# fukangl/SMG-multimodal-grasping

Hardware: AMD Instinct MI355X
Metric: affordance fwd+bwd passes/sec (16-rot 224^2 RGB-D) (higher is better)
Workload: dtype f32; 1 GPU; 16 rot x 224^2 (S=640): fwd + Huber + bwd + Adam per GPU per step; reinforcement_net style 0; 17 trunk passes; fp32; leg=headline, rotations=16, input_size=640, parallelism=dp1

## Files before the change

smg-multimodal-grasping_amd/csrc/backward.hip:

```cpp
#include "engine.h"

int do_backward(smg_engine* e, const smg_net* net, const float* dq, hipStream_t st, int phases, bool elem_head) {
    if (!e->have_fwd) return fail(-22, "smg_backward without a preceding smg_forward");
    if (!net->grads) return fail(-22, "net.grads is NULL");
    if (phases == 2 && !e->bw_phase0_done)
        return fail(-22, "smg_backward_phase(1) must follow smg_backward_phase(0) of the same forward");
    if ((phases & 1) && e->bw_phase0_done)
        return fail(-22, "smg_backward / smg_backward_phase(0) while the second half of a two-phase backward is still due (run phase 1 or a new forward)");
    const Layout& L = *e->L;
    const TrunkRef& T = L.trunk[e->f_trunk];
    const HeadRef& Hd = L.head[e->f_head];
    const int NS = e->f_streams, NP = e->f_pairs;
    const float* P = net->params;
    float* Gr = net->grads;
    const Plane p4 = e->p_blk[3];
    const bool ph_a = phases & 1, ph_b = phases & 2;
    if (ph_a) {
        for (int r = 0; r < kStatRep; ++r) HIP_OK(hipMemsetAsync(e->bstat + (size_t)r * kStatRepStride, 0, 2 * e->bstat_span * sizeof(double), st));
    }
    const bool split16 = e->prec == 0 && kSplitOp == 3;
    if (ph_a && split16) HIP_OK(hipMemsetAsync(e->gamax, 0, (size_t)e->gamax_words * sizeof(unsigned), st));
    const hipStream_t s2 = (e->prof || e->serialize) ? st : e->side;
    auto fork = [&](hipEvent_t ev) -> int {
        HIP_OK(hipEventRecord(ev, st));
// ... 52 lines not shown
        p.bbuf = e->F; p.ldb = 2 * kFeat; p.pb = p4; p.NB = 2 * kFeat;
        p.bsum = fsum(e, e->st_F); p.bsq = fsq(e, e->st_F); p.bstride = 2 * kFeat; p.bgamma = P + Hd.n0.w; p.bbeta = P + Hd.n0.b;
        p.eps = kEps; p.chunk = chunk4; p.chunks_per_stream = cps4; p.n_chunks = NP * cps4;
        p.dw = Gr + Hd.c0.w; p.ldw_out = 2 * kFeat;
        if (fork(e->ev_misc)) return -5;
        const dim3 grid(1, 2 * kFeat / 64, NP * cps4);
        return launch_wgrad(e, s2, p, grid, K_HW0, 2.0 * NP * p4.HW * 2 * kFeat * kHeadMid,
                            4.0 * NP * p4.HW * (2 * kHeadMid + 2 * kFeat), 1, C_IDENT, tiles, tiles.place_alone(wgrad_partial_floats(p, grid)));
        };
        PREC_DISPATCH(e, if (int rc = go(PTAG)) return rc);
    }
    {
        auto run = [&](auto tag, auto ptag) {
                using Cfg = decltype(tag);
                BwdDataP<Cfg, false, E_STORE, true, decltype(ptag)::value, true> p{};
        p.gbuf = e->DH1; p.ldg = kHeadMid; p.gcoff = 0; p.xbuf = e->H1; p.ldx = kHeadMid; p.xcoff = 0; p.pa = p4; p.KA = kHeadMid;
        p.xsum = fsum(e, e->st_H1); p.xsq = fsq(e, e->st_H1); p.xstride = kHeadMid;
        p.s1 = b1(e, e->st_H1); p.s2 = b2(e, e->st_H1); p.sstride = kHeadMid; p.scoff = 0; p.agamma = P + Hd.n1.w;
        p.wp = e->packed_u + e->pk_hd0; p.K8tot = kHeadMid / 8; p.ldn = 2 * kFeat; p.wcol0 = 0; p.N = 2 * kFeat;
        p.mbuf = e->F; p.ldm = 2 * kFeat; p.mcoff = 0; p.pm = p4;
        p.msum = fsum(e, e->st_F); p.msq = fsq(e, e->st_F); p.mstride = 2 * kFeat; p.egamma = P + Hd.n0.w; p.ebeta = P + Hd.n0.b;
        p.dst = e->DF; p.ldd = 2 * kFeat; p.dcoff = 0;
        p.o1 = b1(e, e->st_F); p.o2 = b2(e, e->st_F); p.ostride = 2 * kFeat; p.ocoff = 0;
        p.dbeta = Gr + Hd.n0.b; p.dgamma = Gr + Hd.n0.w; p.rep_stride = 0; p.eps = kEps;
        launch_gemm(e, st, p, dim3(NP * p4.HWp / Cfg::BM, 2 * kFeat / Cfg::BN), K_HD0, 2.0 * NP * p4.HW * 2 * kFeat * kHeadMid,
                    4.0 * NP * p4.HW * (2 * kHeadMid + 2 * 2 * kFeat));
            };
            PREC_DISPATCH(e, if (p4.HWp % 128 == 0) run(CfgP128x128{}, PTAG); else run(CfgP64x128{}, PTAG));
    }
    {
        Norm5BwdArgs a;
        a.DF = e->DF; a.F = e->F; a.p4 = p4; a.fsum = fsum(e, e->st_F); a.fsq = fsq(e, e->st_F);
        a.f1 = b1(e, e->st_F); a.f2 = b2(e, e->st_F); a.hgamma = P + Hd.n0.w;
        a.x4 = e->X[3]; a.xsum = fsum(e, e->st_X[3]); a.xsq = fsq(e, e->st_X[3]); a.gamma5 = P + T.norm5.w; a.eps = kEps;
        a.user_ptr = e->d_user_ptr; a.user_pair = e->d_user_pair; a.user_slot = e->d_user_slot;
        a.G4 = e->G[3]; a.SA = b1(e, e->st_X[3]); a.SB = b2(e, e->st_X[3]);
        a.dbeta5 = Gr + T.norm5.b; a.dgamma5 = Gr + T.norm5.w; a.chunk = 16;
        PREC_DISPATCH(e, launch_kernel(e, norm5_bwd_kernel<PREC>, dim3(4, NS, (p4.HW + 15) / 16), dim3(256), 0, st, K_OTHER, 0, 0, false, a));
    }
    }
    struct LayerBuf { float* GS; float* D2; float* D2S; int ring; };
    auto buf_of = [&](int b, int i) -> LayerBuf {
        const int r = ring_pos(b, i);
        return LayerBuf{e->GS[r % kRing], e->D2[r % kRing], e->D2S[r % kRing], r};
    };
    auto fused_gsrc = [&](int b, const DenseLayerRef& d) {
        const int Ct = kBlockCtot[b];
        GradSrc g{};
        g.g = el(e, e->G[b], d.cin); g.ldg = Ct; g.x = el(e, e->X[b], d.cin); g.ldx = Ct;
        g.xsum = fsum(e, e->st_X[b]) + d.cin; g.xsq = fsq(e, e->st_X[b]) + d.cin;
        g.s1 = b1(e, e->st_X[b]) + d.cin; g.s2 = b2(e, e->st_X[b]) + d.cin; g.sstride = Ct; g.eps = kEps;
        return g;
    };
    auto issue_wgrads = [&](int b, int i) -> int {
        const Plane pl = e->p_blk[b];
        const int Ct = kBlockCtot[b];
        const DenseLayerRef& d = T.layers[b][i];
        float* bt = el(e, e->Bt, e->bt_off[b][i]);
        const LayerBuf lb = buf_of(b, i);
        const WgradPlan w = plan_layer_wgrads(pl, d.cin, NS, e->prec, split16, e->deterministic, e->part_floats, e->generic3x3, e->generic_w1);
        GradSrc gsrc{};
        if (gs_on_side(pl)) launch_gs_apply(b, i, s2, lb.GS);
        if (gs_materialised) { gsrc.g = lb.GS; gsrc.ldg = kGrowth; gsrc.amax = gamax_of(e, b, i, 0); }
        else gsrc = fused_gsrc(b, d);
        if (!e->generic3x3) {
            const PartialTiles::Slot at = tiles.place_halo3x3(w.w3.groups);
            if (at.refused) return fail(-12, tiles.refusal());
            launch_reduce2(e, s2, at.first);
            Halo3x3WgradArgs a;
            a.g = gsrc; a.pl = pl; a.src = bt; a.C = kBottleneck;
            a.bt = bn_table(e, e->sb_tab[b][i], e->max_streams, 0, kBottleneck, P + d.n2.w, P + d.n2.b);
            a.asc = asc_n2(e, b, i);
            a.tiles_x = w.w3.tiles_x; a.n_tiles = w.w3.n_tiles; a.tiles_per_wg = w.w3.tiles_per_wg;
            a.part = part_at(e, at);
            a.groups = w.w3.groups; a.streams = NS;
            const double flops = 2.0 * NS * pl.HW * 9 * kBottleneck * kGrowth, bytes = ESZ(e) * NS * pl.HW * (kGrowth + kBottleneck);
            if (w.w3.ts == 16) {
                PREC_DISPATCH(e, launch_kernel(e, conv3x3_halo_wgrad_kernel<16, PREC>, dim3(w.w3_grid), dim3(256), HaloWgradSGeo<16, PREC>::smem_bytes(), s2,
                                               K_W3, flops, bytes, false, a));
            } else {
                PREC_DISPATCH(e, launch_kernel(e, conv3x3_halo_wgrad_kernel<8, PREC>, dim3(w.w3_grid), dim3(256), HaloWgradSGeo<8, PREC>::smem_bytes(), s2,
                                               K_W3, flops, bytes, false, a));
            }
            launch_reduce2(e, s2, tiles.launched(at, reduce_tap_inner(a.part, w.w3.groups * NS, Gr + d.c2.w)));
        } else {
            int chunk, cps;
            pick_chunk(pl, NS, 9, chunk, cps);
            BwdWeightP<CfgW32x128, W_THREE, C_3x3, kPdWgrad, false> p{};
            p.gbuf = lb.GS; p.ldg = kGrowth; p.gcoff = 0; p.xbuf = nullptr; p.pa = pl; p.MA = kGrowth;
            p.bbuf = bt; p.ldb = kBottleneck; p.pb = pl; p.NB = kBottleneck;
            p.bsum = fsum(e, e->st_Bt[b][i]); p.bsq = fsq(e, e->st_Bt[b][i]); p.bstride = kBottleneck;
            p.bgamma = P + d.n2.w; p.bbeta = P + d.n2.b; p.eps = kEps;
            p.chunk = chunk; p.chunks_per_stream = cps; p.n_chunks = NS * cps;
            p.dw = Gr + d.c2.w; p.ldw_out = kBottleneck * 9;
            const dim3 grid(1, 1, 9 * NS * cps);
            if (int rc = launch_wgrad(e, s2, p, grid, K_W3, 2.0 * NS * pl.HW * 9 * kBottleneck * kGrowth,
                                      ESZ(e) * NS * pl.HW * (kGrowth + kBottleneck), 9, C_3x3, tiles, tiles.place_alone(wgrad_partial_floats(p, grid)))) return rc;
        }
        if (w.w1_ws) {
            using G = WswGeo;
            static_assert(G::BN == kW1WsTileN, "plan_layer_wgrads counts this kernel's column tiles");
            Wgrad1x1WsArgs a{};
            a.d2 = reinterpret_cast<const u32x4*>(lb.D2); a.binv = lb.D2S; a.x = e->X[b]; a.ldb = Ct; a.pl = pl; a.NB = d.cin;
            a.btab = stat_table(e, e->sx_tab[b], e->max_streams, Ct); a.bgamma = P + d.n1.w; a.bbeta = P + d.n1.b; a.basc = asc_n1(e, b, i);
            a.chunk = w.chunk; a.chunks_per_stream = w.cps; a.n_chunks = NS * w.cps;
            a.dw = Gr + d.c1.w; a.ldw_out = d.cin; a.ldp = w.nt * G::BN;
            const PartialTiles::Slot at = tiles.place_behind3x3((int64_t)a.n_chunks * G::BM * a.ldp);
            launch_reduce2(e, s2, at.first);
            if (at.refused) return fail(-12, tiles.refusal());
            a.part = part_at(e, at);
            a.tm = TileMap{a.n_chunks, w.nt, 0};
            launch_kernel(e, conv1x1_wgrad_ws_kernel, dim3(tile_grid(a.tm)), dim3(512), G::smem_bytes(w.chunk), s2, K_W1,
                          2.0 * NS * pl.HW * d.cin * kBottleneck, 4.0 * NS * pl.HW * (kBottleneck + d.cin), false, a);
            ReduceArgs red1{};
            if (a.part) red1 = reduce_chunk_major(a.part, a.n_chunks, 1, G::BM, d.cin, G::BM, a.ldp, a.dw, d.cin, C_IDENT);
            launch_reduce2(e, s2, tiles.launched(at, red1));
        } else {
            using Cfg = CfgW128x64;
            static_assert(Cfg::BN == kW1TileN, "plan_layer_wgrads counts this kernel's column tiles");
            auto go = [&](auto ptag) -> int {
                BwdWeightP<MC<Cfg, decltype(ptag)::value>, W_ONE, C_IDENT, kPdWgrad, false, decltype(ptag)::value> p{};
                p.gbuf = lb.D2; p.ldg = kBottleneck; p.gcoff = 0; p.xbuf = nullptr; p.pa = pl; p.MA = kBottleneck; p.binv = lb.D2S; p.basc = asc_n1(e, b, i);
                p.bbuf = e->X[b]; p.ldb = Ct; p.pb = pl; p.NB = d.cin;
                p.bsum = fsum(e, e->st_X[b]); p.bsq = fsq(e, e->st_X[b]); p.bstride = Ct; p.btab = stat_table(e, e->sx_tab[b], e->max_streams, Ct);
                p.bgamma = P + d.n1.w; p.bbeta = P + d.n1.b; p.eps = kEps;
                p.chunk = w.chunk; p.chunks_per_stream = w.cps; p.n_chunks = NS * w.cps;
                p.dw = Gr + d.c1.w; p.ldw_out = d.cin;
                const dim3 grid(1, w.nt, NS * w.cps);
                return launch_wgrad(e, s2, p, grid, K_W1, 2.0 * NS * pl.HW * d.cin * kBottleneck,
                                    ESZ(e) * NS * pl.HW * (kBottleneck + d.cin), 1, C_IDENT, tiles, tiles.place_behind3x3(wgrad_partial_floats(p, grid)));
            };
            PREC_DISPATCH(e, if (int rc = go(PTAG)) return rc);
        }
        return 0;
    };
    auto debug_stop = [&]() -> int {
        launch_reduce2(e, s2, tiles.drain());
        HIP_OK(hipEventRecord(e->ev_end, s2));
        HIP_OK(hipStreamWaitEvent(st, e->ev_end, 0));
        if (int rc = walk_status(e)) return rc;
        e->have_fwd = false; e->bw_phase0_done = false; e->prof_stage = -1;
        return 0;
    };
    const bool pooled_tail = e->prec == 0 && e->f_stem1 && !e->stem_plane_tail && (NS > 4 || e->deterministic);
    for (int b = ph_a ? 3 : 0; b >= (ph_b ? 0 : 1); --b) {
        e->prof_stage = b;
        const Plane pl = e->p_blk[b];
        const int Ct = kBlockCtot[b];
        if (e->dbg_stop == b * 100 + 50) return debug_stop();
        if (b == 0 && pooled_tail) {
            StemMomArgs a;
            a.img = e->img4; a.pi = e->p_img; a.ps = e->p_stem; a.part = e->mom_part;
// ... 27 lines not shown
                const double flops = 2.0 * NS * pl.HW * 9 * kBottleneck * kGrowth;
                const double bytes = ESZ(e) * NS * pl.HW * (kGrowth + 2 * kBottleneck);
                if (halo_tile(pl, NS) == 16) {
                    a.tiles_x = (pl.W + 15) / 16; a.cg_per_wg = kBottleneck / 32;
                    if (pl.H % 16 || pl.W % 16) {
                        PREC_DISPATCH(e, launch_kernel(e, conv3x3_halo_dgrad_kernel<16, PREC, true>, dim3(((pl.H + 15) / 16) * a.tiles_x, NS), dim3(256),
                                                       HaloDgradSGeo<16, PREC>::smem_bytes(kBottleneck), st, K_D3, flops, bytes, true, a));
                    } else {
                        PREC_DISPATCH(e, launch_kernel(e, conv3x3_halo_dgrad_kernel<16, PREC>, dim3((pl.H / 16) * a.tiles_x, NS), dim3(256),
                                                       HaloDgradSGeo<16, PREC>::smem_bytes(kBottleneck), st, K_D3, flops, bytes, true, a));
                    }
                } else {
                    a.tiles_x = (pl.W + 7) / 8; a.cg_per_wg = 1;
                    PREC_DISPATCH(e, launch_kernel(e, conv3x3_halo_dgrad_kernel<8, PREC>, dim3(((pl.H + 7) / 8) * a.tiles_x, NS, kBottleneck / 64), dim3(256),
                                                   HaloDgradSGeo<8, PREC>::smem_bytes(kBottleneck), st, K_D3, flops, bytes, true, a));
                }
            } else {
                auto run = [&](auto tag) {
                    using Cfg = decltype(tag);
                    BwdDataP<Cfg, true, E_STORE, false> p{};
                    p.gbuf = GSb; p.ldg = kGrowth; p.gcoff = 0; p.xbuf = nullptr; p.pa = pl; p.KA = kGrowth;
                    p.wp = e->packed_u + e->pk_g3d[b][i]; p.K8tot = 9 * kGrowth / 8; p.ldn = kBottleneck; p.wcol0 = 0; p.N = kBottleneck;
                    p.mbuf = bt; p.ldm = kBottleneck; p.mcoff = 0; p.pm = pl;
                    p.msum = fsum(e, e->st_Bt[b][i]); p.msq = fsq(e, e->st_Bt[b][i]); p.mstride = kBottleneck;
                    p.egamma = P + d.n2.w; p.ebeta = P + d.n2.b;
                    p.dst = split16 ? e->DY2 : D2b; p.ldd = kBottleneck; p.dcoff = 0;
                    p.o1 = b1(e, e->st_Bt[b][i]); p.o2 = b2(e, e->st_Bt[b][i]); p.ostride = kBottleneck; p.ocoff = 0;
                    p.dbeta = Gr + d.n2.b; p.dgamma = Gr + d.n2.w; p.eps = kEps;
                    launch_gemm(e, st, p, dim3(NS * pl.HWp / Cfg::BM, kBottleneck / Cfg::BN), K_D3, 2.0 * NS * pl.HW * 9 * kBottleneck * kGrowth,
                                ESZ(e) * NS * pl.HW * (kGrowth + 2 * kBottleneck));
                };
                if (pl.HWp % 128 == 0) run(CfgP128x128{}); else run(CfgP64x128{});
            }
            if (split16) {
                BnBwdApplySplitArgs a{};
                a.g = e->DY2; a.x = bt; a.pl = pl;
                a.xsum = fsum(e, e->st_Bt[b][i]); a.xsq = fsq(e, e->st_Bt[b][i]); a.xstride = kBottleneck; a.xtab = !e->generic3x3 ? stat_table(e, e->sb_tab[b][i], e->max_streams, kBottleneck) : StatTab{};
                a.s1 = b1(e, e->st_Bt[b][i]); a.s2 = b2(e, e->st_Bt[b][i]); a.sstride = kBottleneck;
                a.gamma = P + d.n2.w; a.eps = kEps; a.out = reinterpret_cast<u32x4*>(D2b); a.binv = lb.D2S;
                if (!e->generic3x3) { a.dbeta = Gr + d.n2.b; a.dgamma = Gr + d.n2.w; }
                launch_kernel(e, bn_bwd_apply_split_kernel, dim3(pl.HWp / kScaleBlock, NS), dim3(256), 0, st, K_OTHER, 0, 4.0 * NS * pl.HW * 3 * kBottleneck, false, a);
            } else {
                BnBwdApplyArgs a{};
                a.g = D2b; a.ldg = kBottleneck; a.gcoff = 0; a.x = bt; a.ldx = kBottleneck; a.xcoff = 0; a.pl = pl; a.C = kBottleneck;
                a.xsum = fsum(e, e->st_Bt[b][i]); a.xsq = fsq(e, e->st_Bt[b][i]); a.xstride = kBottleneck; a.xtab = !e->generic3x3 ? stat_table(e, e->sb_tab[b][i], e->max_streams, kBottleneck) : StatTab{};
                a.s1 = b1(e, e->st_Bt[b][i]); a.s2 = b2(e, e->st_Bt[b][i]); a.sstride = kBottleneck; a.scoff = 0;
                a.gamma = P + d.n2.w; a.eps = kEps; a.out = D2b; a.ldo = kBottleneck; a.amax = nullptr;
                if (!e->generic3x3) { a.dbeta = Gr + d.n2.b; a.dgamma = Gr + d.n2.w; }
                PREC_DISPATCH(e, launch_kernel(e, bn_bwd_apply_kernel<PREC>, dim3((pl.HWp + bn_apply_rows(PREC) - 1) / bn_apply_rows(PREC), NS), dim3(256), 0, st,
                                               K_OTHER, 0, ESZ(e) * NS * pl.HW * 3 * kBottleneck, false, a));
            }
            if (fork(e->ev_d2[lb.ring % kRing])) return -5;
            if (int rc = issue_wgrads(b, i)) return rc;
            HIP_OK(hipEventRecord(e->ev_side[lb.ring % kRing], s2));
            if (e->dbg_stop == b * 100 + i && e->prec == 0) {
                const int64_t nf = (int64_t)NS * pl.HWp * Ct;
                if (e->dbg_gsnap_floats < nf) {
                    if (e->dbg_gsnap) (void)hipFree(e->dbg_gsnap);
                    e->dbg_gsnap = nullptr; e->dbg_gsnap_floats = 0;
                    HIP_OK(hipMalloc((void**)&e->dbg_gsnap, (size_t)nf * sizeof(float)));
                    e->dbg_gsnap_floats = nf;
                }
                HIP_OK(hipMemcpyAsync(e->dbg_gsnap, e->G[b], (size_t)nf * sizeof(float), hipMemcpyDeviceToDevice, st));
            }
            const int L = (int)T.layers[b].size();
            const int g_lo = i - ((L - 1 - i) % kGroup == kGroup - 1 ? 0 : std::min(i, kGroup - 1 - (L - 1 - i) % kGroup));
            const int cs = T.layers[b][g_lo].cin;
            if (d.cin > cs) {
                auto run = [&](auto tag, auto ptag) {
                    using Cfg = MC<decltype(tag), decltype(ptag)::value>;
                    BwdDataP<Cfg, false, E_ACCUM, false, decltype(ptag)::value> p{};
                    p.gbuf = D2b; p.ldg = kBottleneck; p.gcoff = 0; p.xbuf = nullptr; p.pa = pl; p.KA = kBottleneck; p.binv = lb.D2S;
                    p.wp = e->packed_u + e->pk_d1[b][i]; p.K8tot = kBottleneck / 8; p.ldn = d.cin; p.wcol0 = cs; p.N = d.cin - cs;
                    p.mbuf = e->X[b]; p.ldm = Ct; p.mcoff = cs; p.pm = pl;
                    p.msum = fsum(e, e->st_X[b]); p.msq = fsq(e, e->st_X[b]); p.mstride = Ct; p.mtab = stat_table(e, e->sx_tab[b], e->max_streams, Ct);
                    p.egamma = P + d.n1.w + cs; p.ebeta = P + d.n1.b + cs;
                    p.dst = e->G[b]; p.ldd = Ct; p.dcoff = cs;
                    p.o1 = b1(e, e->st_X[b]); p.o2 = b2(e, e->st_X[b]); p.ostride = Ct; p.ocoff = cs;
                    p.dbeta = e->dbscr + e->db_off[b][i] + cs; p.dgamma = e->dbscr + e->db_off[b][i] + d.cin + cs; p.rep_stride = e->db_total; p.eps = kEps;
                    launch_gemm(e, st, p, dim3(NS * pl.HWp / Cfg::BM, (p.N + Cfg::BN - 1) / Cfg::BN), K_D1, 2.0 * NS * pl.HW * p.N * kBottleneck,
                                ESZ(e) * NS * pl.HW * (kBottleneck + 3.0 * p.N));
                };
                PREC_DISPATCH(e, if (pl.HWp % 128 == 0) run(CfgP128x64{}, PTAG); else run(CfgP64x64{}, PTAG));
            }
            if (i == g_lo) {
                auto run = [&](auto tag, auto ptag) {
                    using Cfg = MC<decltype(tag), decltype(ptag)::value>;
                    BwdDataGroupP<Cfg, decltype(ptag)::value> p{};
                    const int g_hi = L - 1 - ((L - 1 - g_lo) / kGroup) * kGroup;
                    p.nseg = g_hi - g_lo + 1;
                    for (int k = 0; k < p.nseg; ++k) {
                        const DenseLayerRef& dk = T.layers[b][g_lo + k];
                        const LayerBuf lk = buf_of(b, g_lo + k);
                        p.seg[k].g = lk.D2; p.seg[k].wp = e->packed_u + e->pk_d1[b][g_lo + k]; p.seg[k].ldn = dk.cin; p.seg[k].binv = lk.D2S;
                        p.seg[k].gamma = P + dk.n1.w; p.seg[k].beta = P + dk.n1.b;
                        p.seg[k].dbeta = e->dbscr + e->db_off[b][g_lo + k]; p.seg[k].dgamma = e->dbscr + e->db_off[b][g_lo + k] + dk.cin;
                    }
                    p.ldg = kBottleneck; p.pa = pl; p.KA = kBottleneck; p.N = cs;
                    p.mbuf = e->X[b]; p.ldm = Ct;
                    p.msum = fsum(e, e->st_X[b]); p.msq = fsq(e, e->st_X[b]); p.mstride = Ct; p.mtab = stat_table(e, e->sx_tab[b], e->max_streams, Ct);
                    p.dst = e->G[b]; p.ldd = Ct;
                    p.o1 = b1(e, e->st_X[b]); p.o2 = b2(e, e->st_X[b]); p.ostride = Ct; p.rep_stride = e->db_total; p.eps = kEps;
                    launch_gemm(e, st, p, dim3(NS * pl.HWp / Cfg::BM, (cs + Cfg::BN - 1) / Cfg::BN), K_D1, 2.0 * NS * pl.HW * cs * kBottleneck * p.nseg,
                                ESZ(e) * NS * pl.HW * ((double)p.nseg * kBottleneck + 3.0 * cs));
                };
                PREC_DISPATCH(e, if (pl.HWp % 128 == 0) run(GemmCfg<128, 64, 32, 2, 2, 1, true>{}, PTAG); else run(CfgP64x64{}, PTAG));
            }
// ... 139 lines not shown
```

smg-multimodal-grasping_amd/csrc/engine.h:

```cpp
#pragma once
#include <hip/hip_runtime.h>

#include <algorithm>
#include <cmath>
#include <cstdio>
#include <cstdlib>
#include <cstring>
#include <string>
#include <type_traits>
#include <vector>

#include "../../include/smg_hip.h"
#include "elem.cuh"
#include "scene.cuh"
#include "gemm.cuh"
#include "halo.cuh"
#include "ws.cuh"
#include "wsw.cuh"
#include "plan.h"

using namespace smg;

int smg_fail(int code, const std::string& msg);
static inline int fail(int code, const std::string& msg) { return smg_fail(code, msg); }
// ... 42 lines not shown
struct ProfRec { hipEvent_t a, b; int kind; double flops; int stage; double bytes; };

struct StatArr { int64_t off; int stride; };

struct smg_engine {
    int device = 0, S = 0, max_streams = 0, max_pairs = 0, head_out = 1;
    Plane p_img, p_stem, p_blk[4];
    int OH = 1, OW = 1;
    const Layout* L = nullptr;

    float* img4 = nullptr; float* stem = nullptr; float* X[4] = {}; float* Bt = nullptr;
    std::vector<int64_t> bt_off[4];
    unsigned char* argmax = nullptr;
    float* F = nullptr; float* H1 = nullptr;
    float* G[4] = {}; float* GS[kRing] = {}; float* D2[kRing] = {}; float* part = nullptr; int64_t part_floats = 0;
    float* DY2 = nullptr; float* D2S[kRing] = {};
    hipStream_t side = nullptr; hipEvent_t ev_gs[kRing] = {}, ev_d2[kRing] = {}, ev_side[kRing] = {}, ev_misc = nullptr, ev_end = nullptr; float* DY0 = nullptr; float* DH1 = nullptr; float* DF = nullptr;
    double* fstat = nullptr; int64_t fstat_span = 0;
    double* bstat = nullptr; int64_t bstat_span = 0;
    float* dbscr = nullptr; int db_total = 0; int db_off[4][24] = {}; int db_toff[3] = {}; struct DbSeg* d_dbseg = nullptr; int n_dbseg = 0;
    StatArr st_stem, st_X[4], st_F, st_H1; std::vector<StatArr> st_Bt[4];
    u32x4* packed_u = nullptr; int64_t packed_units = 0;
    float* packed_f = nullptr; int64_t packed_floats = 0;
    PackDesc* d_pack = nullptr; std::vector<PackDesc> h_pack[3]; std::vector<PackDesc> h_pack_head[3];
    int pack_stride = 0, bnupd_stride = 0, n_bnupd = 0;
    int64_t pk_conv0 = 0, pk_conv0_1 = 0, pk_head0 = 0, pk_hd0 = 0, pk_head1 = 0;
    std::vector<int64_t> pk_c1[4], pk_d1[4], pk_g3f[4], pk_g3d[4], pk_hf[4], pk_hd[4]; int64_t pk_t[3] = {}, pk_td[3] = {};
    int max_pack = 0;
    float* asc = nullptr; ActScaleDesc* d_asc = nullptr; int n_asc = 0;
    unsigned* gamax = nullptr; int64_t gamax_words = 0;
    float* stab = nullptr; int64_t stab_floats = 0;
    int64_t sx_tab[4] = {}, sb_tab[4][24] = {}, sf_tab = 0;
    BnUpdDesc* d_bnupd = nullptr;
    bool have_fwd = false; int f_trunk = 0, f_head = 0, f_streams = 0, f_pairs = 0;
    bool bw_phase0_done = false;
    bool f_dense_dq = false;
    int head_bwd = 0;
    bool f_stem1 = false;
    int* d_stream_image = nullptr; int* d_stream_rot = nullptr; int* d_pair_a = nullptr; int* d_pair_b = nullptr;
    int* d_seq_t = nullptr; int* d_seq_h = nullptr; int* d_user_ptr = nullptr; int* d_user_pair = nullptr; int* d_user_slot = nullptr;
    float* d_affine = nullptr;
    float* scene_val = nullptr; int* scene_idx = nullptr; int scene_tiles = 0;
    double* scene_lpart = nullptr;
    double* scene_gpart = nullptr; int* scene_cnt = nullptr;
    int* d_stage = nullptr; int* h_stage[2] = {}; hipEvent_t ev_stage[2] = {}; int stage_ints = 0, stage_turn = 0;
    int so_image = 0, so_rot = 0, so_pa = 0, so_pb = 0, so_seq_t = 0, so_seq_h = 0, so_uptr = 0, so_upair = 0, so_uslot = 0, so_aff = 0, so_ma = 0, so_mb = 0, so_adam = 0;
    bool capturing = false; int* h_stage_g = nullptr; hipEvent_t ev_graph = nullptr, ev_gin = nullptr; hipStream_t gstream = nullptr; struct StepGraph* step_graph = nullptr;
    int64_t workspace_bytes = 0;
    int n_cu = 256;
    int prec = 0;
    bool serialize = false;
    bool deterministic = false;
    bool generic3x3 = false, generic_c1 = false, generic_w1 = false, stem_plane_tail = false;
    float* stemv = nullptr; float* mom_part = nullptr; double* mom = nullptr; int mom_groups = 0;
    int dbg_stop = -1;
    float* dbg_gsnap = nullptr; int64_t dbg_gsnap_floats = 0;
    bool prof = false; std::vector<ProfRec> recs; std::vector<hipEvent_t> ev_pool;
    double prof_ms[5][K_COUNT] = {}; int64_t prof_n[5][K_COUNT] = {}; double prof_flops[5][K_COUNT] = {}; double prof_bytes[5][K_COUNT] = {}; int prof_stage = -1;
    int launch_rc = 0;
};

constexpr int kMomTilesPerWg = 8;
static inline int stem_mom_tiles_x(const Plane& ps) { return (ps.W + kMomT - 1) / kMomT; }
static inline int stem_mom_tiles(const Plane& ps) { return stem_mom_tiles_x(ps) * ((ps.H + kMomT - 1) / kMomT); }
static inline int stem_mom_groups(const Plane& ps) { return (stem_mom_tiles(ps) + kMomTilesPerWg - 1) / kMomTilesPerWg; }

static Plane make_plane(int H, int W) {
    Plane p; p.H = H; p.W = W; p.HW = H * W;
    const int g = p.HW >= 8192 ? 128 : 64;
    p.HWp = (p.HW + g - 1) / g * g;
    return p;
}

template <class T>
static int dev_alloc(smg_engine* e, T** out, int64_t count) {
    void* p = nullptr;
    hipError_t err = hipMalloc(&p, (size_t)count * sizeof(T));
    if (err != hipSuccess) return fail(-12, std::string("hipMalloc ") + std::to_string(count * sizeof(T)) + " B: " + hipGetErrorString(err));
    e->workspace_bytes += count * (int64_t)sizeof(T);
    *out = (T*)p;
    return 0;
}
#define ALLOC(ptr, count) do { int _r = dev_alloc(e, &(ptr), (count)); if (_r) return _r; } while (0)

static hipEvent_t prof_event(smg_engine* e) {
    if (!e->ev_pool.empty()) { hipEvent_t ev = e->ev_pool.back(); e->ev_pool.pop_back(); return ev; }
    hipEvent_t ev; (void)hipEventCreate(&ev); return ev;
}
#define ESZ(e) ((e)->prec ? 2.0 : 4.0)
struct ProfScope {
    smg_engine* e; hipStream_t st; int kind; double flops, bytes; hipEvent_t a{}, b{};
    ProfScope(smg_engine* e_, hipStream_t s, int k, double f, double by) : e(e_), st(s), kind(k), flops(f), bytes(by) {
        if (e->prof) { a = prof_event(e); b = prof_event(e); (void)hipEventRecord(a, st); }
    }
    ~ProfScope() {
        if (e->prof) { (void)hipEventRecord(b, st); e->recs.push_back({a, b, kind, flops, e->prof_stage, bytes}); }
    }
};

#define PTAG std::integral_constant<int, PREC>{}
#define PREC_DISPATCH(e, CALL)                                            \
    switch ((e)->prec) {                                                  \
        case 1: { constexpr int PREC = 1; CALL; } break;                  \
        case 2: { constexpr int PREC = 2; CALL; } break;                  \
        default: { constexpr int PREC = 0; CALL; } break;                 \
    }
// ... 166 lines not shown
```

smg-multimodal-grasping_amd/csrc/engine.hip:

```cpp
#include "engine.h"

static thread_local std::string g_err;
int smg_fail(int code, const std::string& msg) { g_err = msg; return code; }

static int engine_build(smg_engine* e) {
    const Layout& L = *e->L;
    const int NS = e->max_streams, NP = e->max_pairs;
    const int S = e->S;
    const int H1 = (S - 1) / 2 + 1, H2 = (H1 - 1) / 2 + 1;
    e->p_img = make_plane(S, S);
    e->p_stem = make_plane(H1, H1);
    int h = H2;
    for (int b = 0; b < 4; ++b) { e->p_blk[b] = make_plane(h, h); h /= 2; }
    e->OH = e->OW = e->p_blk[3].H - kHeadKernel + 1;
    if (e->OH < 1) return fail(-22, "input_size too small for the 20x20 value head");

    if (getenv("SMG_SERIALIZE")) e->serialize = true;
    const int cross = getenv("SMG_CROSSCHECK") ? atoi(getenv("SMG_CROSSCHECK")) : 0;
    e->generic3x3 = cross & 1; e->generic_c1 = cross & 2; e->generic_w1 = cross & 4; e->stem_plane_tail = cross & 8;

    ALLOC(e->img4, (int64_t)NS * e->p_img.HWp * 4);
    ALLOC(e->stem, (int64_t)NS * e->p_stem.HWp * 64);
    ALLOC(e->DY0, (int64_t)NS * e->p_stem.HWp * 64);
    ALLOC(e->argmax, (int64_t)NS * e->p_blk[0].HWp * 64);
    e->stemv = e->DY0;
    e->mom_groups = stem_mom_groups(e->p_stem);
    ALLOC(e->mom_part, (int64_t)NS * e->mom_groups * kMomVals);
    ALLOC(e->mom, (int64_t)NS * kMomOut);
    int64_t bt_total = 0;
    for (int b = 0; b < 4; ++b) {
        ALLOC(e->X[b], (int64_t)NS * e->p_blk[b].HWp * kBlockCtot[b]);
        ALLOC(e->G[b], (int64_t)NS * e->p_blk[b].HWp * kBlockCtot[b]);
        for (int i = 0; i < kBlockLayers[b]; ++i) {
            e->bt_off[b].push_back(bt_total);
            bt_total += (int64_t)NS * e->p_blk[b].HWp * kBottleneck;
        }
    }
    ALLOC(e->Bt, bt_total);
    for (int k = 0; k < kRing; ++k) {
        ALLOC(e->D2[k], (int64_t)NS * e->p_blk[0].HWp * kBottleneck);
        ALLOC(e->GS[k], (int64_t)NS * e->p_blk[0].HWp * kGrowth);
        ALLOC(e->D2S[k], (int64_t)NS * (e->p_blk[0].HWp / kScaleBlock));
        HIP_OK(hipEventCreateWithFlags(&e->ev_gs[k], hipEventDisableTiming));
        HIP_OK(hipEventCreateWithFlags(&e->ev_d2[k], hipEventDisableTiming));
        HIP_OK(hipEventCreateWithFlags(&e->ev_side[k], hipEventDisableTiming));
    }
    ALLOC(e->DY2, (int64_t)NS * e->p_blk[0].HWp * kBottleneck);
    e->scene_tiles = (int)(((int64_t)(S / 2) * (S / 2) + kSceneTile - 1) / kSceneTile);
    ALLOC(e->scene_val, (int64_t)kSceneMaps * e->scene_tiles);
    ALLOC(e->scene_idx, (int64_t)kSceneMaps * e->scene_tiles);
    ALLOC(e->scene_lpart, (int64_t)kSceneMaps * e->OH * e->OW);
    ALLOC(e->scene_gpart, (int64_t)kSceneMaps * e->OH * e->OW * 3);
    ALLOC(e->scene_cnt, (int64_t)kSceneMaps * e->OH * e->OW);
    HIP_OK(hipEventCreateWithFlags(&e->ev_misc, hipEventDisableTiming));
    HIP_OK(hipEventCreateWithFlags(&e->ev_end, hipEventDisableTiming));
    HIP_OK(hipStreamCreateWithFlags(&e->side, hipStreamNonBlocking));
    e->part_floats = (int64_t)24 << 20;
    for (int b = 0; b < 4; ++b) {
        const Plane& pl = e->p_blk[b];
        for (int ts : {halo_tile(pl), 8})
            e->part_floats = std::max(e->part_floats, w3_partial_floats(w3_tiling(pl, ts, NS, INT64_MAX).groups, NS));
    }
    ALLOC(e->part, e->part_floats);
    ALLOC(e->F, (int64_t)NP * e->p_blk[3].HWp * 2 * kFeat);
    ALLOC(e->DF, (int64_t)NP * e->p_blk[3].HWp * 2 * kFeat);
    ALLOC(e->H1, (int64_t)NP * e->p_blk[3].HWp * kHeadMid);
    ALLOC(e->DH1, (int64_t)NP * e->p_blk[3].HWp * kHeadMid);

    int64_t off = 0;
    auto carve = [&](int n, int stride) { StatArr s{off, stride}; off += (int64_t)n * stride; return s; };
    e->st_stem = carve(NS, 64);
    for (int b = 0; b < 4; ++b) e->st_X[b] = carve(NS, kBlockCtot[b]);
// ... 878 lines not shown
```

smg-multimodal-grasping_amd/csrc/wgrad_plan.h:

```cpp
#pragma once
#include <cstdint>
#include <string>

#include "plan.h"

namespace smg {

struct Plane { int H, W, HW, HWp; };

enum { C_IDENT = 0, C_3x3 = 1, C_STEM = 2, C_STEM1 = 3 };

struct ReduceArgs {
    const float* part; int Z, taps, rows, cols, ldp; int64_t z_stride, tap_stride;
    float* dw; int ldw_out, cmap;
};
static inline ReduceArgs reduce_chunk_major(const float* part, int n_chunks, int taps, int rows, int cols, int64_t rows_padded, int64_t ldp,
                                            float* dw, int ldw_out, int cmap) {
    ReduceArgs r{};
    r.part = part; r.Z = n_chunks; r.taps = taps; r.rows = rows; r.cols = cols; r.ldp = (int)ldp;
    r.z_stride = rows_padded * ldp; r.tap_stride = (int64_t)n_chunks * rows_padded * ldp;
    r.dw = dw; r.ldw_out = ldw_out; r.cmap = cmap;
    return r;
}
static inline ReduceArgs reduce_tap_inner(const float* part, int n_tiles, float* dw) {
// ... 3 lines not shown
    r.dw = dw; r.ldw_out = kBottleneck * 9; r.cmap = C_3x3;
    return r;
}
struct ReducePair {
    ReduceArgs a{}, b{};
    static int blocks(const ReduceArgs& r) { return r.Z ? (r.taps * r.rows * r.cols + 63) / 64 : 0; }
};

static inline void pick_chunk(const Plane& pl, int n_planes, int tiles_per_chunk, int& chunk, int& cps, int target = 768) {
    const int want = (target + tiles_per_chunk - 1) / tiles_per_chunk;
    cps = (want + n_planes - 1) / n_planes;
    if (cps < 1) cps = 1;
    chunk = ((pl.HW + cps - 1) / cps + 63) / 64 * 64;
    cps = (pl.HW + chunk - 1) / chunk;
}

static inline int halo_tile(const Plane& p, int n_streams = 1 << 20) {
    return (int64_t)((p.H + 15) / 16) * ((p.W + 15) / 16) * n_streams >= 200 ? 16 : 8;
}

static inline int64_t w3_partial_floats(int groups, int n_streams) { return (int64_t)groups * n_streams * 9 * 32 * kBottleneck; }

static inline int w3_tiles_per_wg(int n_tiles, int ts, int n_streams, int64_t part_floats, double fix_scale = 1.0) {
    const double fix = (ts == 16 ? 0.6 : 2.4) * fix_scale;
    double best = 1e30;
    int tpw_best = 1;
    for (int tpw = 1; tpw <= n_tiles; ++tpw) {
        const int g = (n_tiles + tpw - 1) / tpw;
        const int rounds = (g * (kBottleneck / 32) * n_streams + 511) / 512;
        const double cost = rounds * (tpw + fix);
        if (cost < best - 1e-9) { best = cost; tpw_best = tpw; }
    }
    while (tpw_best < n_tiles && w3_partial_floats((n_tiles + tpw_best - 1) / tpw_best, n_streams) > part_floats) ++tpw_best;
    return tpw_best;
}

constexpr int kW3TileH = 8;
struct W3Tiling { int ts, tiles_x, n_tiles, tiles_per_wg, groups; };
static inline W3Tiling w3_tiling(const Plane& pl, int ts, int n_streams, int64_t part_floats) {
    W3Tiling t;
    t.ts = ts;
    t.tiles_x = (pl.W + ts - 1) / ts; t.n_tiles = ((pl.H + kW3TileH - 1) / kW3TileH) * t.tiles_x;
    t.tiles_per_wg = w3_tiles_per_wg(t.n_tiles, ts, n_streams, part_floats, (double)ts / kW3TileH);
    t.groups = (t.n_tiles + t.tiles_per_wg - 1) / t.tiles_per_wg;
    return t;
}

constexpr int kW1WsTileN = 128, kW1TileN = 64;

struct WgradPlan {
    W3Tiling w3; unsigned w3_grid;
    bool w1_ws; int nt, chunk, cps;
};
static inline WgradPlan plan_layer_wgrads(const Plane& pl, int cin, int NS, int prec, bool split16, bool deterministic, int64_t part_floats,
                                          bool generic3x3, bool generic_w1) {
    WgradPlan w{};
    if (!generic3x3) {
        w.w3 = w3_tiling(pl, halo_tile(pl, NS), NS, part_floats);
        w.w3_grid = (unsigned)(((w.w3.groups * NS + 7) / 8) * 8 * (kBottleneck / 32));
    }
    w.w1_ws = split16 && !generic_w1 && cin > 64 && (deterministic || NS > 4);
    if (w.w1_ws) {
        w.nt = (cin + kW1WsTileN - 1) / kW1WsTileN;
        pick_chunk(pl, NS, w.nt, w.chunk, w.cps, 320);
    } else {
        w.nt = (cin + kW1TileN - 1) / kW1TileN;
        pick_chunk(pl, NS, w.nt, w.chunk, w.cps, (prec && NS >= 16) ? 160 : (NS <= 4 && !deterministic) ? 128 : 320);
    }
    return w;
}

class PartialTiles {
public:
    enum Kind { ALONE, HALO3, HALO3_PAIRED, BEHIND3 };
    struct Slot {
        Kind kind; int64_t off;
        int64_t size;
        ReducePair first;
        bool refused;
    };
    PartialTiles(int64_t floats_, int n_streams, bool deterministic_) : floats(floats_), NS(n_streams), deterministic(deterministic_) {}

    Slot place_alone(int64_t need) {
        Slot s{ALONE, need <= floats ? 0 : -1, need, drain(), false};
        if (s.off < 0 && deterministic) s.refused = refuse(need, floats);
        return s;
    }
    Slot place_halo3x3(int groups) {
        Slot s{HALO3, 0, w3_partial_floats(groups, NS), ReducePair{}, false};
        if (s.size > floats) { s.refused = refuse(-1, floats); return s; }
        if (!deterministic && NS <= 4 && s.size * 2 <= floats) s.kind = HALO3_PAIRED;
        if (s.kind == HALO3) s.first = drain();
        else if (half) s.off = floats / 2;
        return s;
    }
    Slot place_behind3x3(int64_t need) {
        Slot s{BEHIND3, cursor, need, ReducePair{}, false};
        const bool partial = deterministic || NS > 4;
        if (held.Z && (!partial || s.off + need > floats)) { s.first.a = held; held.Z = 0; s.off = 0; }
        const int64_t have = floats - s.off;
        if (!partial || need > have) s.off = -1;
        if (partial && s.off < 0 && deterministic) s.refused = refuse(need, have);
        return s;
    }
    ReducePair launched(const Slot& s, const ReduceArgs& r) {
        ReducePair due;
        if (s.kind == ALONE) due.a = r;
        else if (s.kind == BEHIND3) { due.a = held; due.b = r; held.Z = 0; cursor = 0; }
        else if (s.kind == HALO3) { held = r; cursor = s.size; }
        else {
            if (carried.Z) { due.a = carried; due.b = r; carried.Z = 0; }
            else carried = r;
            half ^= 1;
        }
        return due;
    }
    ReducePair drain() { ReducePair due; due.a = carried; carried.Z = 0; return due; }
    std::string refusal() const {
        if (refusal_need < 0) return "partial-gradient workspace too small";
        return "deterministic: a weight-gradient launch needs " + std::to_string(refusal_need) + " partial-tile floats, the workspace holds " +
               std::to_string(refusal_have);
    }

private:
    bool refuse(int64_t need, int64_t have) { refusal_need = need; refusal_have = have; return true; }
    int64_t floats; int NS; bool deterministic;
    ReduceArgs carried{};
    ReduceArgs held{};
    int64_t cursor = 0;
    int half = 0;
    int64_t refusal_need = 0, refusal_have = 0;
};

}
```

smg-multimodal-grasping_amd/csrc/wsw.cuh:

```cuda
#pragma once
#include "gemm.cuh"

namespace smg {

struct Wgrad1x1WsArgs {
    const u32x4* d2; const float* binv;
    const float* x; int ldb; Plane pl; int NB;
    StatTab btab; const float* bgamma; const float* bbeta; const float* basc;
    int chunk, chunks_per_stream, n_chunks;
    float* dw; int ldw_out;
    float* part; int ldp;
    TileMap tm;
};

struct WswGeo {
    static constexpr int BM = 128, BN = 128, BK = 32;
    static constexpr int PLANE = BK + 4;
    static constexpr int LDTB = BN + 32;
    static constexpr int A_BYTES = 2 * (BM / 8) * PLANE * 16, B_BYTES = 2 * BK * LDTB * 2;
    static constexpr int A_N = 2 * (BM / 8) * BK / 256, B_N = BK * (BN / 4) / 256;
    static constexpr int TILE_BYTES = 2 * (A_BYTES + B_BYTES);
    __host__ __device__ static constexpr int smem_bytes(int chunk) { return TILE_BYTES + (3 * BN + chunk / kScaleBlock + 1) * 4; }
};

// ... 129 lines not shown
#pragma unroll
                for (int j = 0; j < 2; ++j)
#pragma unroll
                    for (int r = 0; r < 16; ++r) acc[i][j][r] *= f;
            cur_inv = inv;
        }
    };
    if (role == 0) {
        int kt = 0;
        for (; kt + 2 <= KT; kt += 2) {
            if (!skip) compute(0);
            rescale(kt);
            __syncthreads();
            if (!skip) compute(1);
            rescale(kt + 1);
            __syncthreads();
        }
        if (kt < KT) { if (!skip) compute(0); __syncthreads(); }
    } else {
        g_load(KT > 2 ? 2 : KT - 1, ra[0], rb[0]);
        int kt = 0;
        for (; kt + 2 <= KT; kt += 2) {
            s_store(1, ra[1], rb[1]);
            g_load(kt + 3 < KT ? kt + 3 : KT - 1, ra[1], rb[1]);
            __syncthreads();
            s_store(0, ra[0], rb[0]);
            g_load(kt + 4 < KT ? kt + 4 : KT - 1, ra[0], rb[0]);
            __syncthreads();
        }
        if (kt < KT) __syncthreads();
        return;
    }

    const float gi = cur_inv * a.basc[1];
    const int l31 = lane & 31;
#pragma unroll
    for (int i = 0; i < 2; ++i)
#pragma unroll
        for (int j = 0; j < 2; ++j) {
            const int col = n0 + wn0 + j * 32 + l31;
            if (a.part) {
                if (col >= a.NB) continue;
                float* ob = a.part + ((int64_t)z * G::BM + wm0 + i * 32 + 4 * half) * a.ldp + col;
#pragma unroll
                for (int r = 0; r < 16; ++r) ob[(int64_t)((r & 3) + 8 * (r >> 2)) * a.ldp] = acc[i][j][r] * gi;
            } else if (col < a.NB) {
                float* ob = a.dw + (int64_t)(wm0 + i * 32 + 4 * half) * a.ldw_out + col;
#pragma unroll
                for (int r = 0; r < 16; ++r) atomicAdd(ob + (int64_t)((r & 3) + 8 * (r >> 2)) * a.ldw_out, acc[i][j][r] * gi);
            }
        }
}

}
```

Measured before the change: 62.97 passes/s.

## Pair adjacent dense layers' 1x1 weight-gradient kernels into one shared-input launch

Adds a paired variant of the warp-specialised 1x1 weight-gradient kernel that handles two consecutive dense layers in one 1024-thread workgroup. The shared input activations X are loaded and staged once per tile, and each layer's gradient is accumulated by its own half of the compute waves. The backward schedule assigns pair roles so the second layer skips its own launch, defers its partial reduction, and the side-stream events are recorded for both ring slots. The aim is to halve launches and X reads for large planes, at the cost of more LDS (near the per-CU limit), one workgroup per CU, and a reordered reduction and event schedule.

```diff
diff --git a/smg-multimodal-grasping_amd/csrc/backward.hip b/smg-multimodal-grasping_amd/csrc/backward.hip
--- a/smg-multimodal-grasping_amd/csrc/backward.hip
+++ b/smg-multimodal-grasping_amd/csrc/backward.hip
@@ -128,13 +128,23 @@
         g.s1 = b1(e, e->st_X[b]) + d.cin; g.s2 = b2(e, e->st_X[b]) + d.cin; g.sstride = Ct; g.eps = kEps;
         return g;
     };
+    const int w1_pair = e->w1_pair;
+    auto plan_of = [&](int b, int i) {
+        return plan_layer_wgrads(e->p_blk[b], T.layers[b][i].cin, NS, e->prec, split16, e->deterministic, e->part_floats, e->generic3x3, e->generic_w1, w1_pair);
+    };
+    int w1_role[4][24] = {};
+    for (int b = 0; b < 4; ++b)
+        w1_pair_roles((int)T.layers[b].size(), [&](int lo, int hi) {
+            return e->dbg_stop != b * 100 + hi &&
+                   w1_pair_fits(e->p_blk[b], plan_of(b, lo), plan_of(b, hi), NS, e->deterministic, e->part_floats, e->generic3x3, w1_pair);
+        }, w1_role[b]);
     auto issue_wgrads = [&](int b, int i) -> int {
         const Plane pl = e->p_blk[b];
         const int Ct = kBlockCtot[b];
         const DenseLayerRef& d = T.layers[b][i];
         float* bt = el(e, e->Bt, e->bt_off[b][i]);
         const LayerBuf lb = buf_of(b, i);
-        const WgradPlan w = plan_layer_wgrads(pl, d.cin, NS, e->prec, split16, e->deterministic, e->part_floats, e->generic3x3, e->generic_w1);
+        const WgradPlan w = plan_of(b, i);
         GradSrc gsrc{};
         if (gs_on_side(pl)) launch_gs_apply(b, i, s2, lb.GS);
         if (gs_materialised) { gsrc.g = lb.GS; gsrc.ldg = kGrowth; gsrc.amax = gamax_of(e, b, i, 0); }
@@ -173,7 +183,38 @@
             if (int rc = launch_wgrad(e, s2, p, grid, K_W3, 2.0 * NS * pl.HW * 9 * kBottleneck * kGrowth,
                                       ESZ(e) * NS * pl.HW * (kGrowth + kBottleneck), 9, C_3x3, tiles, tiles.place_alone(wgrad_partial_floats(p, grid)))) return rc;
         }
-        if (w.w1_ws) {
+        if (w.w1_ws && w1_role[b][i] > 0) {
+            launch_reduce2(e, s2, tiles.defer_behind3x3());
+        } else if (w.w1_ws && w1_role[b][i] < 0) {
+            using G = WswGeo;
+            using GP = WswPairGeo;
+            static_assert(GP::TILE_BYTES == kW1PairLdsTile && G::BN == kW1WsTileN && G::BM == kBottleneck, "w1_pair_fits counts this kernel's LDS and tiles");
+            Wgrad1x1WsPairArgs a{};
+            a.x = e->X[b]; a.ldb = Ct; a.pl = pl; a.btab = stat_table(e, e->sx_tab[b], e->max_streams, Ct);
+            a.chunk = w.chunk; a.chunks_per_stream = w.cps; a.n_chunks = NS * w.cps; a.ldp = w.nt * G::BN;
+            const int64_t tiles1 = (int64_t)a.n_chunks * G::BM * a.ldp;
+            const PartialTiles::Slot at = tiles.place_behind3x3(2 * tiles1);
+            launch_reduce2(e, s2, at.first);
+            if (at.refused) return fail(-12, tiles.refusal());
+            ReduceArgs red[kWswPair] = {};
+            double cols = 0;
+            for (int k = 0; k < kWswPair; ++k) {
+                const DenseLayerRef& dk = T.layers[b][i + k];
+                const LayerBuf lk = buf_of(b, i + k);
+                WswPairLayer& l = a.l[k];
+                l.d2 = reinterpret_cast<const u32x4*>(lk.D2); l.binv = lk.D2S; l.NB = dk.cin;
+                l.bgamma = P + dk.n1.w; l.bbeta = P + dk.n1.b; l.basc = asc_n1(e, b, i + k);
+                l.dw = Gr + dk.c1.w; l.ldw_out = dk.cin;
+                l.part = at.off >= 0 ? part_at(e, at) + k * tiles1 : nullptr;
+                if (l.part) red[k] = reduce_chunk_major(l.part, a.n_chunks, 1, G::BM, dk.cin, G::BM, a.ldp, l.dw, dk.cin, C_IDENT);
+                cols += dk.cin;
+            }
+            a.tm = TileMap{a.n_chunks, w.nt, 0};
+            launch_kernel(e, conv1x1_wgrad_ws_kernel_pair, dim3(tile_grid(a.tm)), dim3(1024), GP::smem_bytes(w.chunk), s2, K_W1,
+                          2.0 * NS * pl.HW * cols * kBottleneck, 4.0 * NS * pl.HW * (kWswPair * kBottleneck + T.layers[b][i + 1].cin), false, a);
+            launch_reduce2(e, s2, tiles.launched(at, red[0]));
+            launch_reduce2(e, s2, ReducePair{red[1], ReduceArgs{}});
+        } else if (w.w1_ws) {
             using G = WswGeo;
             static_assert(G::BN == kW1WsTileN, "plan_layer_wgrads counts this kernel's column tiles");
             Wgrad1x1WsArgs a{};
@@ -307,7 +348,8 @@
             }
             if (fork(e->ev_d2[lb.ring % kRing])) return -5;
             if (int rc = issue_wgrads(b, i)) return rc;
-            HIP_OK(hipEventRecord(e->ev_side[lb.ring % kRing], s2));
+            if (w1_role[b][i] <= 0) HIP_OK(hipEventRecord(e->ev_side[lb.ring % kRing], s2));
+            if (w1_role[b][i] < 0) HIP_OK(hipEventRecord(e->ev_side[buf_of(b, i + 1).ring % kRing], s2));
             if (e->dbg_stop == b * 100 + i && e->prec == 0) {
                 const int64_t nf = (int64_t)NS * pl.HWp * Ct;
                 if (e->dbg_gsnap_floats < nf) {
diff --git a/smg-multimodal-grasping_amd/csrc/engine.h b/smg-multimodal-grasping_amd/csrc/engine.h
--- a/smg-multimodal-grasping_amd/csrc/engine.h
+++ b/smg-multimodal-grasping_amd/csrc/engine.h
@@ -118,6 +118,7 @@
     bool serialize = false;
     bool deterministic = false;
     bool generic3x3 = false, generic_c1 = false, generic_w1 = false, stem_plane_tail = false;
+    int w1_pair = W1PAIR_AUTO;
     float* stemv = nullptr; float* mom_part = nullptr; double* mom = nullptr; int mom_groups = 0;
     int dbg_stop = -1;
     float* dbg_gsnap = nullptr; int64_t dbg_gsnap_floats = 0;
diff --git a/smg-multimodal-grasping_amd/csrc/engine.hip b/smg-multimodal-grasping_amd/csrc/engine.hip
--- a/smg-multimodal-grasping_amd/csrc/engine.hip
+++ b/smg-multimodal-grasping_amd/csrc/engine.hip
@@ -18,6 +18,7 @@
     if (getenv("SMG_SERIALIZE")) e->serialize = true;
     const int cross = getenv("SMG_CROSSCHECK") ? atoi(getenv("SMG_CROSSCHECK")) : 0;
     e->generic3x3 = cross & 1; e->generic_c1 = cross & 2; e->generic_w1 = cross & 4; e->stem_plane_tail = cross & 8;
+    e->w1_pair = (cross & 32) ? W1PAIR_OFF : (cross & 16) ? W1PAIR_ON : W1PAIR_AUTO;
 
     ALLOC(e->img4, (int64_t)NS * e->p_img.HWp * 4);
     ALLOC(e->stem, (int64_t)NS * e->p_stem.HWp * 64);
diff --git a/smg-multimodal-grasping_amd/csrc/wgrad_plan.h b/smg-multimodal-grasping_amd/csrc/wgrad_plan.h
--- a/smg-multimodal-grasping_amd/csrc/wgrad_plan.h
+++ b/smg-multimodal-grasping_amd/csrc/wgrad_plan.h
@@ -79,14 +79,17 @@
     W3Tiling w3; unsigned w3_grid;
     bool w1_ws; int nt, chunk, cps;
 };
+enum { W1PAIR_AUTO = 0, W1PAIR_ON = 1, W1PAIR_OFF = 2 };
+constexpr int kW1PairMinHW = 6400;
+constexpr int kW1PairLdsTile = 155648, kLdsPerCu = 160 * 1024;
 static inline WgradPlan plan_layer_wgrads(const Plane& pl, int cin, int NS, int prec, bool split16, bool deterministic, int64_t part_floats,
-                                          bool generic3x3, bool generic_w1) {
+                                          bool generic3x3, bool generic_w1, int w1_pair = W1PAIR_AUTO) {
     WgradPlan w{};
     if (!generic3x3) {
         w.w3 = w3_tiling(pl, halo_tile(pl, NS), NS, part_floats);
         w.w3_grid = (unsigned)(((w.w3.groups * NS + 7) / 8) * 8 * (kBottleneck / 32));
     }
-    w.w1_ws = split16 && !generic_w1 && cin > 64 && (deterministic || NS > 4);
+    w.w1_ws = split16 && !generic_w1 && cin > 64 && (deterministic || NS > 4 || w1_pair == W1PAIR_ON);
     if (w.w1_ws) {
         w.nt = (cin + kW1WsTileN - 1) / kW1WsTileN;
         pick_chunk(pl, NS, w.nt, w.chunk, w.cps, 320);
@@ -95,6 +98,26 @@
         pick_chunk(pl, NS, w.nt, w.chunk, w.cps, (prec && NS >= 16) ? 160 : (NS <= 4 && !deterministic) ? 128 : 320);
     }
     return w;
+}
+static inline bool w1_pair_fits(const Plane& pl, const WgradPlan& lo, const WgradPlan& hi, int NS, bool deterministic, int64_t part_floats,
+                                bool generic3x3, int w1_pair) {
+    if (w1_pair == W1PAIR_OFF || !lo.w1_ws || !hi.w1_ws) return false;
+    if (w1_pair == W1PAIR_AUTO && !(pl.HW >= kW1PairMinHW && NS > 4)) return false;
+    if (lo.nt != hi.nt || lo.chunk != hi.chunk || lo.cps != hi.cps) return false;
+    if (kW1PairLdsTile + 2 * (3 * kW1WsTileN + lo.chunk / 64 + 1) * 4 > kLdsPerCu) return false;
+    if (deterministic || NS > 4) {
+        const int64_t tiles1 = (int64_t)NS * lo.cps * kBottleneck * lo.nt * kW1WsTileN;
+        if ((generic3x3 ? 0 : w3_partial_floats(lo.w3.groups, NS)) + 2 * tiles1 > part_floats) return false;
+    }
+    return true;
+}
+template <class Ok>
+static inline void w1_pair_roles(int L, Ok ok, int* role) {
+    for (int i = 0; i < L; ++i) role[i] = 0;
+    for (int u = L - 1; u > 0;) {
+        if (ok(u - 1, u)) { role[u] = 1; role[u - 1] = -1; u -= 2; }
+        else u -= 1;
+    }
 }
 
 class PartialTiles {
@@ -142,6 +165,7 @@
         }
         return due;
     }
+    ReducePair defer_behind3x3() { ReducePair due; due.a = held; held.Z = 0; cursor = 0; return due; }
     ReducePair drain() { ReducePair due; due.a = carried; carried.Z = 0; return due; }
     std::string refusal() const {
         if (refusal_need < 0) return "partial-gradient workspace too small";
diff --git a/smg-multimodal-grasping_amd/csrc/wsw.cuh b/smg-multimodal-grasping_amd/csrc/wsw.cuh
--- a/smg-multimodal-grasping_amd/csrc/wsw.cuh
+++ b/smg-multimodal-grasping_amd/csrc/wsw.cuh
@@ -205,4 +205,223 @@
         }
 }
 
+constexpr int kWswPair = 2;
+struct WswPairLayer {
+    const u32x4* d2; const float* binv; int NB;
+    const float* bgamma; const float* bbeta; const float* basc;
+    float* dw; int ldw_out; float* part;
+};
+struct Wgrad1x1WsPairArgs {
+    WswPairLayer l[kWswPair];
+    const float* x; int ldb; Plane pl; StatTab btab;
+    int chunk, chunks_per_stream, n_chunks; int ldp;
+    TileMap tm;
+};
+
+struct WswPairGeo {
+    using G = WswGeo;
+    static constexpr int A_N = 2 * (G::BM / 8) * G::BK / 512, B_N = G::BK * (G::BN / 4) / 512;
+    static constexpr int TILE_BYTES = kWswPair * G::TILE_BYTES;
+    __host__ __device__ static constexpr int smem_bytes(int chunk) { return TILE_BYTES + kWswPair * (3 * G::BN + chunk / kScaleBlock + 1) * 4; }
+};
+
+static __global__ __launch_bounds__(1024, 1) void conv1x1_wgrad_ws_kernel_pair(const Wgrad1x1WsPairArgs a) {
+    using G = WswGeo;
+    using GP = WswPairGeo;
+    extern __shared__ __attribute__((aligned(16))) float smem[];
+    char* As = reinterpret_cast<char*>(smem);
+    char* Bs = As + 2 * kWswPair * G::A_BYTES;
+    float* bp = reinterpret_cast<float*>(As + GP::TILE_BYTES);
+    float* sinv0 = bp + kWswPair * 3 * G::BN;
+    const int t = threadIdx.x, role = t >> 9, tp = t & 511, lane = t & 63, wave = (t >> 6) & 3, half = lane >> 5;
+    const int layer = sgpr((t >> 8) & 1);
+    int z, nt;
+    tile_decode(a.tm, blockIdx.x, z, nt);
+    const int n = sgpr(z / a.chunks_per_stream);
+    const int p0 = sgpr((z - n * a.chunks_per_stream) * a.chunk);
+    if (p0 >= a.pl.HW) return;
+    const int n0 = sgpr(nt * G::BN);
+    int len = a.pl.HWp - p0;
+    len = len < a.chunk ? len : a.chunk;
+    const int KT = sgpr(len / G::BK);
+    const int n_sinv = a.chunk / kScaleBlock + 1;
+
+    const float* xn = a.x + (int64_t)n * a.pl.HWp * a.ldb;
+    const unsigned d2_bytes = 16u * (unsigned)(2 * kD2K8 * a.pl.HWp), x_bytes = 4u * (unsigned)(a.pl.HW * a.ldb);
+    unsigned a_voff[GP::A_N], b_voff[GP::B_N];
+#pragma unroll
+    for (int i = 0; i < GP::A_N; ++i) {
+        const int id = tp + 512 * i, kr = id % G::BK, q = id / G::BK;
+        a_voff[i] = 16u * (unsigned)(q * a.pl.HWp + kr);
+    }
+    const int bq = tp % (G::BN / 4), bl = tp / (G::BN / 4);
+#pragma unroll
+    for (int i = 0; i < GP::B_N; ++i) b_voff[i] = 4u * (unsigned)((bl + 16 * i) * a.ldb + n0 + 4 * bq);
+    u32x4 ra[2][kWswPair][GP::A_N]; float4 rb[2][GP::B_N];
+    auto g_load = [&](int kt, u32x4 (&xa)[kWswPair][GP::A_N], float4 (&xb)[GP::B_N]) {
+#pragma unroll
+        for (int l = 0; l < kWswPair; ++l)
+#pragma unroll
+            for (int i = 0; i < GP::A_N; ++i)
+                xa[l][i] = bload_u4(a.l[l].d2 + d2_stream_units(n, a.pl.HWp), d2_bytes, a_voff[i], 16u * (unsigned)(p0 + kt * G::BK));
+#pragma unroll
+        for (int i = 0; i < GP::B_N; ++i) xb[i] = bload4(xn, x_bytes, b_voff[i], 4u * (unsigned)((p0 + kt * G::BK) * a.ldb));
+    };
+    KPrm3 bfix[kWswPair] = {};
+    auto s_store = [&](int buf, const u32x4 (&xa)[kWswPair][GP::A_N], const float4 (&xb)[GP::B_N]) {
+#pragma unroll
+        for (int l = 0; l < kWswPair; ++l) {
+            char* A = As + (buf * kWswPair + l) * G::A_BYTES;
+            char* B = Bs + (buf * kWswPair + l) * G::B_BYTES;
+#pragma unroll
+            for (int i = 0; i < GP::A_N; ++i) {
+                const int id = tp + 512 * i;
+                *reinterpret_cast<u32x4*>(A + ((id / G::BK) * G::PLANE + id % G::BK) * 16) = xa[l][i];
+            }
+#pragma unroll
+            for (int i = 0; i < GP::B_N; ++i) {
+                const Split4 s = split4<3>(bnrelu4<true>(xb[i], bfix[l]));
+                const int kr = bl + 16 * i;
+#pragma unroll
+                for (int pc = 0; pc < 2; ++pc) *reinterpret_cast<uint2*>(B + ((pc * G::BK + kr) * G::LDTB + 4 * bq) * 2) = s.p[pc];
+            }
+        }
+    };
+    if (role == 1) {
+        g_load(0, ra[0], rb[0]);
+        g_load(KT > 1 ? 1 : 0, ra[1], rb[1]);
+    }
+    if (t < kWswPair * G::BN) {
+        const int l = sgpr(t / G::BN), c = t % G::BN, ch = n0 + c;
+        const WswPairLayer& L = a.l[l];
+        float mean = 0.f, sc = 0.f, be = 0.f;
+        if (ch < L.NB) {
+            const float sa = L.basc[0];
+            mean = a.btab.mean[(int64_t)n * a.btab.ld + ch];
+            sc = L.bgamma[ch] * a.btab.invstd[(int64_t)n * a.btab.ld + ch] * sa;
+            be = L.bbeta[ch] * sa;
+        }
+        float* b = bp + l * 3 * G::BN;
+        b[c] = mean; b[G::BN + c] = sc; b[2 * G::BN + c] = be;
+    }
+#pragma unroll
+    for (int l = 0; l < kWswPair; ++l) {
+        const float* bi = a.l[l].binv + (int64_t)n * (a.pl.HWp / kScaleBlock) + p0 / kScaleBlock;
+        for (int j = t; j * kScaleBlock < KT * G::BK; j += 1024) sinv0[l * n_sinv + j] = bi[j];
+    }
+    __syncthreads();
+    if (role == 1) {
+#pragma unroll
+        for (int l = 0; l < kWswPair; ++l) {
+            const float* b = bp + l * 3 * G::BN;
+            bfix[l].mean = ldv4(b + 4 * bq); bfix[l].scale = ldv4(b + G::BN + 4 * bq); bfix[l].beta = ldv4(b + 2 * G::BN + 4 * bq);
+        }
+        s_store(0, ra[0], rb[0]);
+    }
+    __syncthreads();
+
+    const float* sinv = sinv0 + layer * n_sinv;
+    f32x16 acc[2][2];
+#pragma unroll
+    for (int i = 0; i < 2; ++i)
+#pragma unroll
+        for (int j = 0; j < 2; ++j)
+#pragma unroll
+            for (int r = 0; r < 16; ++r) acc[i][j][r] = 0.f;
+    const int wm0 = (wave >> 1) * 64, wn0 = (wave & 1) * 64;
+    const int tr_row = (lane & 15) >> 2, tr_col = ((lane >> 4) & 1) * 16 + (lane & 3) * 4;
+    auto tr2 = [&](const char* p, int stride) -> u32x4 {
+        const u32x2 lo = __builtin_bit_cast(u32x2, __builtin_amdgcn_ds_read_tr16_b64_v4i16((lds_s16x4*)p));
+        const u32x2 hi = __builtin_bit_cast(u32x2, __builtin_amdgcn_ds_read_tr16_b64_v4i16((lds_s16x4*)(p + stride)));
+        return u32x4{lo.x, lo.y, hi.x, hi.y};
+    };
+    auto compute = [&](int buf) {
+        const char* A = As + (buf * kWswPair + layer) * G::A_BYTES;
+        const char* B = Bs + (buf * kWswPair + layer) * G::B_BYTES;
+#pragma unroll
+        for (int s = 0; s < G::BK / 16; ++s) {
+            const int k0 = s * 16 + 8 * half + tr_row;
+            u32x4 af[2][2], bf[2][2];
+#pragma unroll
+            for (int pc = 0; pc < 2; ++pc)
+#pragma unroll
+                for (int i = 0; i < 2; ++i) {
+                    const int ch = wm0 + i * 32 + tr_col;
+                    af[pc][i] = tr2(A + ((pc * (G::BM / 8) + (ch >> 3)) * G::PLANE + k0) * 16 + ((ch >> 2) & 1) * 8, 4 * 16);
+                    bf[pc][i] = tr2(B + ((pc * G::BK + k0) * G::LDTB + wn0 + i * 32 + tr_col) * 2, 4 * G::LDTB * 2);
+                }
+#pragma unroll
+            for (int g = 0; g < 3; ++g)
+#pragma unroll
+                for (int i = 0; i < 2; ++i)
+#pragma unroll
+                    for (int j = 0; j < 2; ++j) acc[i][j] = mfma_f16(af[g == 1 ? 1 : 0][i], bf[g == 0 ? 1 : 0][j], acc[i][j]);
+        }
+    };
+    constexpr int kSkipBinades = 64;
+    float cur_inv = sinv[0];
+    bool skip = false;
+    auto rescale = [&](int kt) {
+        const int nx = (kt + 1) * G::BK;
+        if (nx % kScaleBlock || kt + 1 >= KT) return;
+        const float inv = sinv[nx / kScaleBlock];
+        skip = cur_inv != 1.f && (int)(__float_as_uint(cur_inv) >> 23) - (int)(__float_as_uint(inv) >> 23) >= kSkipBinades;
+        if (inv != cur_inv && !skip) {
+            const float f = cur_inv * __uint_as_float((254u << 23) - __float_as_uint(inv));
+#pragma unroll
+            for (int i = 0; i < 2; ++i)
+#pragma unroll
+                for (int j = 0; j < 2; ++j)
+#pragma unroll
+                    for (int r = 0; r < 16; ++r) acc[i][j][r] *= f;
+            cur_inv = inv;
+        }
+    };
+    if (role == 0) {
+        int kt = 0;
+        for (; kt + 2 <= KT; kt += 2) {
+            if (!skip) compute(0);
+            rescale(kt);
+            __syncthreads();
+            if (!skip) compute(1);
+            rescale(kt + 1);
+            __syncthreads();
+        }
+        if (kt < KT) { if (!skip) compute(0); __syncthreads(); }
+    } else {
+        g_load(KT > 2 ? 2 : KT - 1, ra[0], rb[0]);
+        int kt = 0;
+        for (; kt + 2 <= KT; kt += 2) {
+            s_store(1, ra[1], rb[1]);
+            g_load(kt + 3 < KT ? kt + 3 : KT - 1, ra[1], rb[1]);
+            __syncthreads();
+            s_store(0, ra[0], rb[0]);
+            g_load(kt + 4 < KT ? kt + 4 : KT - 1, ra[0], rb[0]);
+            __syncthreads();
+        }
+        if (kt < KT) __syncthreads();
+        return;
+    }
+
+    const WswPairLayer& L = a.l[layer];
+    const float gi = cur_inv * L.basc[1];
+    const int l31 = lane & 31;
+#pragma unroll
+    for (int i = 0; i < 2; ++i)
+#pragma unroll
+        for (int j = 0; j < 2; ++j) {
+            const int col = n0 + wn0 + j * 32 + l31;
+            if (col >= L.NB) continue;
+            if (L.part) {
+                float* ob = L.part + ((int64_t)z * G::BM + wm0 + i * 32 + 4 * half) * a.ldp + col;
+#pragma unroll
+                for (int r = 0; r < 16; ++r) ob[(int64_t)((r & 3) + 8 * (r >> 2)) * a.ldp] = acc[i][j][r] * gi;
+            } else {
+                float* ob = L.dw + (int64_t)(wm0 + i * 32 + 4 * half) * L.ldw_out + col;
+#pragma unroll
+                for (int r = 0; r < 16; ++r) atomicAdd(ob + (int64_t)((r & 3) + 8 * (r >> 2)) * L.ldw_out, acc[i][j][r] * gi);
+            }
+        }
 }
+
+}
```

New measurement: 63.54 passes/s (median of 6 runs). About the same (+0.9%).
